# cbg-ethz/LongSom

Measured on AMD Instinct MI355X. Metric: genomic sites/s pileup+call, 10M-read BAM x 5k barcodes, 1/2/4/8 MI355X, higher is better.
Workload: dtype u32

## Files before the change

### longsom_amd/csrc/lsg_api.hip

```cpp
#include "lsg_ctx.h"
#include <cstdarg>
#include <cstring>

namespace lsg {
static thread_local char g_err[512] = "";
void set_error(const char* fmt, ...) {
    va_list ap; va_start(ap, fmt); vsnprintf(g_err, sizeof(g_err), fmt, ap); va_end(ap);
}
const char* get_error() { return g_err; }

int run_count(lsg_ctx* c, const lsg_count_params* p);
int run_fetch_counts(lsg_ctx* c, int ct, int64_t* keys, uint8_t* ref, uint32_t* counts, int64_t capacity);
int run_call(lsg_ctx* c, const lsg_call_params* p);
int run_fetch_calls(lsg_ctx* c, lsg_call* out, int64_t capacity, int candidates_only, int64_t* n_out);
int run_select_calls(lsg_ctx* c, int kind, lsg_call* dst_device, int64_t capacity, int64_t* n_out);
int run_probe(lsg_ctx* c, int kind, const int64_t* keys, int64_t n, uint8_t* hits, int on_device);
int run_set_table_names(lsg_ctx* c, int32_t n_contigs, const char* contig_names, int32_t n_ct, const char* ct_names);
int run_format_table(lsg_ctx* c, int32_t table, int64_t* n_bytes);
int run_copy_table(lsg_ctx* c, int32_t table, char* dst, int64_t capacity);
int run_append_table(lsg_ctx* c, int32_t table, const char* path);
int run_free_table(lsg_ctx* c, int32_t table);
int run_step2_summary(lsg_ctx* c, int32_t n_cols, uint8_t* kinds, int64_t* n_survivor_bytes);
int run_genotype(lsg_ctx* c, const lsg_genotype_params* p, int64_t n_sites, const int64_t* site_keys, const uint8_t* alt_sym,
                 uint32_t* dp, uint32_t* alt, int on_device, int32_t max_depth, int64_t n_groups, const int64_t* group_off);
// ... 35 lines not shown

int lsg_create(int device_id, lsg_ctx** out) {
    if (!out) { set_error("lsg_create: out is NULL"); return -2; }
    *out = nullptr;
    int n = 0;
    if (hipGetDeviceCount(&n) != hipSuccess || n <= 0) {
        set_error("lsg_create: no HIP device visible (this library has no CPU fallback)");
        return -1;
    }
    if (device_id < 0 || device_id >= n) { set_error("lsg_create: device %d out of range [0,%d)", device_id, n); return -2; }
    LSG_HIP(hipSetDevice(device_id));
    lsg_ctx* c = new lsg_ctx();
    c->device = device_id;
    { hipDeviceProp_t prop; if (hipGetDeviceProperties(&prop, device_id) == hipSuccess && prop.multiProcessorCount > 0) c->n_cus = prop.multiProcessorCount; }
    if (hipStreamCreateWithFlags(&c->copy_stream, hipStreamNonBlocking) != hipSuccess || hipEventCreateWithFlags(&c->ev_copy, hipEventDisableTiming) != hipSuccess || hipEventCreateWithFlags(&c->ev_blk, hipEventDisableTiming) != hipSuccess || hipEventCreateWithFlags(&c->ev_lpt, hipEventDisableTiming) != hipSuccess ||
        hipStreamCreateWithFlags(&c->own_stream, hipStreamNonBlocking) != hipSuccess) {
        set_error("lsg_create: hipStreamCreate failed"); delete c; return -1;
    }
    c->stream = c->own_stream;
    if (hipHostMalloc(reinterpret_cast<void**>(&c->h_pin), 4096, hipHostMallocDefault) != hipSuccess) { set_error("lsg_create: hipHostMalloc failed"); delete c; return -1; }
    for (auto& e : c->ev)
        if (hipEventCreate(&e) != hipSuccess) { set_error("lsg_create: hipEventCreate failed"); delete c; return -1; }
    for (auto& e : c->evb)
        if (hipEventCreate(&e) != hipSuccess) { set_error("lsg_create: hipEventCreate failed"); delete c; return -1; }
    *out = c;
    return 0;
}

void lsg_destroy(lsg_ctx* c) {
    if (!c) return;
// ... 11 lines not shown
    for (auto& b : c->syn) b.release();
    for (auto& b : c->gen) b.release();
    (void)run_free_table(c, -1);
    c->cg.release();
    c->tab_names.release();
    for (auto& b : c->ws) b.release();
    for (auto& b : c->tm) b.release();
    for (auto& b : c->bt) b.release();
    for (auto& e : c->ev) if (e) (void)hipEventDestroy(e);
    for (auto& e : c->evb) if (e) (void)hipEventDestroy(e);
    if (c->own_stream) (void)hipStreamDestroy(c->own_stream);
    if (c->copy_stream) (void)hipStreamDestroy(c->copy_stream);
    if (c->ev_copy) (void)hipEventDestroy(c->ev_copy);
    if (c->ev_blk) (void)hipEventDestroy(c->ev_blk);
    if (c->ev_lpt) (void)hipEventDestroy(c->ev_lpt);
    if (c->h_pin) (void)hipHostFree(c->h_pin);
    delete c;
}

int lsg_unload_reads(lsg_ctx* c) {
    if (!c) { set_error("lsg_unload_reads: NULL handle"); return -2; }
    LSG_HIP(hipSetDevice(c->device));
    LSG_HIP(hipStreamSynchronize(c->stream));
    DevBuf* bufs[] = {&c->b_read_tid, &c->b_read_pos, &c->b_read_flag, &c->b_read_mapq, &c->b_read_cb, &c->b_seg_read, &c->b_seg_start, &c->b_seg_len,
                      &c->b_seg_ev_off, &c->b_events, &c->d_read_key, &c->d_read_drop, &c->d_read_adm, &c->d_ne_units, &c->d_ne_mask, &c->d_ne_rowbase, &c->d_ne_rowoff,
                      &c->d_cub_tmp, &c->d_ix_stat, &c->d_tile_cap, &c->d_tile_off, &c->d_calls, &c->d_site_off, &c->d_pass_list, &c->d_defer_list};
    for (auto* b : bufs) b->release();
    for (auto& b : c->d_rows) b.release();
    for (auto& b : c->gen) b.release();
    for (auto& b : c->ws) b.release();
// ... 436 lines not shown
```

### longsom_amd/csrc/lsg_ctx.h

```cpp
#pragma once
#include <hip/hip_runtime.h>
#include <cstdint>
#include <cstdio>
#include <string>
#include <vector>
#include "../../include/longsom_hip.h"
#include "../../include/longsom_synth.h"

namespace lsg {

constexpr int TILE_W = 64;
constexpr int ROW_PLANES = 34;
constexpr int NCTR = 33;

constexpr int ROW_QUADS = (ROW_PLANES + 3) / 4;
constexpr uint64_t ROW_BLOCK_WORDS = (uint64_t)ROW_QUADS * 256;
constexpr uint64_t ROW_STORED_WORDS = (uint64_t)ROW_QUADS * 4;
constexpr uint32_t ROW_NARROW = 1u << 31;
__host__ __device__ inline uint64_t row_word(uint64_t row, int plane) {
    return (row >> 6) * ROW_BLOCK_WORDS + (uint64_t)(plane >> 2) * 256 + (row & 63) * 4 + (uint64_t)(plane & 3);
}

void set_error(const char* fmt, ...);
const char* get_error();
// ... 66 lines not shown
__global__ void k_read_end(const uint32_t* seg_read, const int32_t* seg_start, const int32_t* seg_len, int64_t n_segs, int32_t* read_end);
__global__ void k_read_end_init(const int32_t* read_pos, int64_t n_reads, int32_t* read_end);
int depth_cap_drops(lsg_ctx* c, const lsg_count_params* p);
struct GatherCountSrc { const uint16_t* events; int64_t n_events; const uint64_t* key; const uint32_t* rdv; int32_t cb_bits; int32_t src_shift; int32_t wsh; };
int run_gather_count(lsg_ctx* c, const lsg_count_params* p, const GatherCountSrc& src, bool direct);
}

struct lsg_ctx {
    int device = 0;
    hipStream_t stream = nullptr;
    hipStream_t own_stream = nullptr;
    hipStream_t copy_stream = nullptr;
    hipEvent_t ev_copy = nullptr;
    hipEvent_t ev_blk = nullptr;
    hipEvent_t ev_lpt = nullptr;
    hipEvent_t ev[6] = {nullptr, nullptr, nullptr, nullptr, nullptr, nullptr};
    hipEvent_t evb[5] = {nullptr, nullptr, nullptr, nullptr, nullptr};

    int32_t n_contigs = 0;
    std::vector<int64_t> contig_len;
    std::vector<uint32_t> tile_base;
    uint32_t n_tiles = 0;
    uint32_t tile_lo = 0, tile_hi = 0;
    lsg::DevBuf d_tile_base, d_contig_len, d_ref_ptrs;
    std::vector<lsg::DevBuf> ref;
    std::vector<const uint8_t*> ref_ptr;

    int32_t n_cb = 0, n_ct = 0;
    lsg::DevBuf d_celltype_of, d_ct_rank;
    std::vector<uint8_t> h_celltype_of;
// ... 85 lines not shown
```

### longsom_amd/csrc/pileup.hip

```cpp
#include "lsg_ctx.h"
#include <hipcub/hipcub.hpp>
#include <cstdio>
#include <cstdlib>
#include <cstring>

namespace lsg {

#define LSG_AS3 __attribute__((address_space(3)))
__device__ __forceinline__ uint32_t lds_addr(const void* p) { return (uint32_t)(uintptr_t)(LSG_AS3 const void*)p; }
constexpr int ARENA = 256;

enum { SC_COLS = 8, SC_OVERFLOW = 9, SC_READS = 10, SC_SEGS = 11, SC_EVENTS = 12, SC_ROWS_DEEP = 15,
       SC_ROWS = 16, SC_ROWS_SRC = 28, SC_NENT = 38, SC_QWALK = 48,
       SC_ROWALLOC = 160, SC_ROWALLOC_STRIDE = 16, SC_COUNT = SC_ROWALLOC + SC_ROWALLOC_STRIDE * LSG_MAX_CELLTYPES };

struct CountArgs {
    int64_t n_reads;
    const int32_t* read_tid; const uint16_t* read_flag; const uint8_t* read_mapq; const int32_t* read_cb;
    const int64_t* contig_len; const uint8_t* const* ref_ptr;
    const uint8_t* celltype_of;
    int32_t n_contigs, n_cb, n_ct;
    uint32_t tile_lo, tile_hi;
    int32_t min_bq, min_mq, min_dp, min_cc, ignore_orphans;
    uint32_t flag_exclude;
// ... 1139 lines not shown
            __syncthreads();
            const uint32_t nn = rl(s_q[2], 0);
            const int ct = tm.ct_base + wv;
            if (counting && ct < a.n_ct)
                tm_finish<TmCounters>(a, pl + wv * 1024, nc_sh[wv][lane], cj.w0 + ct, cj.slab + (uint32_t)ct * cj.nj, cj.nj, cj.tcnt, ct, cj.tid, cj.tstart, lane, &book, refb, 0);
            if (nxt == XcdQueue::NO_JOB) break;
            cur = nxt; nxt = nn;
        }
    }
    lds_fence();
    __syncthreads();
    stat_flush(tg.stat_slots, stat, lane, wv);
    books_flush(a, books, lane);
}

__device__ __forceinline__ void tw_add(TmState& s0, TmState& s1, uint32_t m, uint32_t ev, uint32_t thr, uint32_t pk0, uint32_t pk1, uint32_t one) {
    const uint32_t r = m;
    if (!TM_ASM) {
        const uint32_t ln = threadIdx.x & 63u;
        auto half = [&](TmState& s, uint32_t e, uint32_t f, uint32_t inv, uint32_t pk) {
            if (m & TMM_CLOSE) { s.nc += s.mask & 0x10001u; s.mask = 0; }
            if (m & TMM_SKIP) return;
            const bool counted = (e & 0xffu) >= thr && ln >= f && ln < 64u - inv;
            if (!counted) return;
            const uint32_t addr = (pk | (e & 0x700u)) + (m & TMM_CT12);
            const uint32_t sym8 = (e >> 8) & 15u, ctone = 1u << ((m >> 8) & 16u);
            uint32_t hi = 1u;
            if (m & TMM_SINGLE) s.nc += ctone;
            else if (m & TMM_FIRST) s.mask = (1u << sym8) | ctone;
            else { hi |= (s.mask & (1u << sym8)) << 5; s.mask |= (1u << sym8) | ctone; }
            __hip_atomic_fetch_add((LSG_AS3 unsigned long long*)(uintptr_t)addr, ((unsigned long long)hi << 32) | ((e & 0xffu) | (m & TMM_FWD)), __ATOMIC_RELAXED, __HIP_MEMORY_SCOPE_WORKGROUP);
        };
        half(s0, ev & 0xffffu, r & 63u, (r >> 6) & 63u, pk0);
        half(s1, ev >> 16, (r >> 13) & 63u, (r >> 21) & 63u, pk1);
        return;
    }
    uint32_t t0, t1, addr, dlo, elo, ehi, sa, sb, sc, st; unsigned long long xm;
#define TW_RANGE0 "s_lshr_b32 %[st], %[r], 6\n\ts_lshl_b64 %[xm], -1, %[r]\n\ts_lshr_b64 exec, -1, %[st]\n\ts_and_b64 exec, exec, %[xm]\n\t"
#define TW_RANGE1 "s_lshr_b32 %[st], %[r], 13\n\ts_lshl_b64 %[xm], -1, %[st]\n\ts_lshr_b32 %[st], %[r], 21\n\ts_lshr_b64 exec, -1, %[st]\n\ts_and_b64 exec, exec, %[xm]\n\t"
#define TW_HEAD(WSEL, BSEL, PK, DLO)                                                                                                 \
        "v_and_b32_sdwa %[addr], %[c700], %[ev] dst_sel:DWORD dst_unused:UNUSED_PAD src0_sel:DWORD src1_sel:" WSEL "\n\t"           \
        "v_or3_b32 %[addr], %[addr], " PK ", %[sa]\n\t"                                                                             \
        "v_or_b32_sdwa " DLO ", %[sb], %[ev] dst_sel:DWORD dst_unused:UNUSED_PAD src0_sel:DWORD src1_sel:" BSEL "\n\t"              \
        "v_cmpx_le_u32_sdwa vcc, %[thr], %[ev] src0_sel:DWORD src1_sel:" BSEL "\n\t"
    asm volatile(
        "s_bitcmp1_b32 %[m], 27\n\t"
        "s_cbranch_scc0 1f\n\t"
        "v_and_b32 %[t0], 0x10001, %[mask0]\n\t"
        "v_and_b32 %[t1], 0x10001, %[mask1]\n\t"
        "v_add_u32 %[nc0], %[nc0], %[t0]\n\t"
        "v_add_u32 %[nc1], %[nc1], %[t1]\n\t"
        "v_mov_b32 %[mask0], 0\n\t"
        "v_mov_b32 %[mask1], 0\n"
        "1:\n\t"
        "s_bitcmp1_b32 %[m], 29\n\t"
        "s_cbranch_scc1 9f\n\t"
        "s_and_b32 %[sa], %[m], 0x1000\n\t"
        "s_and_b32 %[sb], %[m], 0x100000\n\t"
        "s_lshr_b32 %[sc], %[sa], 8\n\t"
        "s_lshl_b32 %[sc], 1, %[sc]\n\t"
        "s_bitcmp1_b32 %[m], 30\n\t"
        "s_cbranch_scc0 2f\n\t"
        TW_RANGE0
        TW_HEAD("WORD_0", "BYTE_0", "%[pk0]", "v92")
        "ds_add_u64 %[addr], v[92:93]\n\t"
        "v_add_u32 %[nc0], %[sc], %[nc0]\n\t"
        TW_RANGE1
        TW_HEAD("WORD_1", "BYTE_2", "%[pk1]", "v92")
        "ds_add_u64 %[addr], v[92:93]\n\t"
        "v_add_u32 %[nc1], %[sc], %[nc1]\n\t"
        "s_branch 8f\n"
        "2:\n\t"
        "s_bitcmp1_b32 %[m], 28\n\t"
        "s_cbranch_scc0 3f\n\t"
        TW_RANGE0
        TW_HEAD("WORD_0", "BYTE_0", "%[pk0]", "v92")
        "v_bfe_u32 %[t1], %[ev], 8, 4\n\t"
        "ds_add_u64 %[addr], v[92:93]\n\t"
        "v_lshl_or_b32 %[mask0], %[one], %[t1], %[sc]\n\t"
        TW_RANGE1
        TW_HEAD("WORD_1", "BYTE_2", "%[pk1]", "v92")
        "v_bfe_u32 %[t1], %[ev], 24, 4\n\t"
        "ds_add_u64 %[addr], v[92:93]\n\t"
        "v_lshl_or_b32 %[mask1], %[one], %[t1], %[sc]\n\t"
        "s_branch 8f\n"
        "3:\n\t"
        TW_RANGE0
        TW_HEAD("WORD_0", "BYTE_0", "%[pk0]", "v94")
        "v_lshlrev_b32_sdwa %[t1], %[ev], %[one] dst_sel:DWORD dst_unused:UNUSED_PAD src0_sel:BYTE_1 src1_sel:DWORD\n\t"
        "v_and_b32 %[t0], %[mask0], %[t1]\n\t"
        "v_lshl_or_b32 v95, %[t0], 5, %[one]\n\t"
        "ds_add_u64 %[addr], v[94:95]\n\t"
        "v_or3_b32 %[mask0], %[mask0], %[t1], %[sc]\n\t"
        TW_RANGE1
        TW_HEAD("WORD_1", "BYTE_2", "%[pk1]", "v94")
        "v_lshlrev_b32_sdwa %[t1], %[ev], %[one] dst_sel:DWORD dst_unused:UNUSED_PAD src0_sel:BYTE_3 src1_sel:DWORD\n\t"
        "v_and_b32 %[t0], %[mask1], %[t1]\n\t"
        "v_lshl_or_b32 v95, %[t0], 5, %[one]\n\t"
        "ds_add_u64 %[addr], v[94:95]\n\t"
        "v_or3_b32 %[mask1], %[mask1], %[t1], %[sc]\n"
        "8:\n\t"
        "s_mov_b64 exec, -1\n"
        "9:"
        : [t0] "=&v"(t0), [t1] "=&v"(t1), [addr] "=&v"(addr), [dlo] "=&{v92}"(dlo), [elo] "=&{v94}"(elo), [ehi] "=&{v95}"(ehi),
          [sa] "=&s"(sa), [sb] "=&s"(sb), [sc] "=&s"(sc), [st] "=&s"(st), [xm] "=&s"(xm),
          [mask0] "+v"(s0.mask), [nc0] "+v"(s0.nc), [mask1] "+v"(s1.mask), [nc1] "+v"(s1.nc)
        : [ev] "v"(ev), [m] "s"(m), [r] "s"(m), [thr] "s"(thr), [c700] "s"(0x700u), [one] "{v93}"(one), [pk0] "v"(pk0), [pk1] "v"(pk1)
        : "scc", "vcc", "memory");
#undef TW_RANGE0
#undef TW_RANGE1
#undef TW_HEAD
}

struct TwCounters {
    const uint32_t* pl; int lane; uint32_t ncdup;
    __device__ __forceinline__ uint32_t lo(int k) const { return pl[(lane & 1) * 2048 + k * 64 + (lane >> 1) * 2]; }
    __device__ __forceinline__ uint32_t hi(int k) const { return pl[(lane & 1) * 2048 + k * 64 + (lane >> 1) * 2 + 1]; }
    __device__ __forceinline__ uint32_t BC(int k) const { return hi(k) & 0x1fffu; }
    __device__ __forceinline__ uint32_t DUP(int k) const { return hi(k) >> (13 + k); }
    __device__ __forceinline__ uint32_t BQ(int k) const { return lo(k) & 0xfffffu; }
    __device__ __forceinline__ uint32_t BCF(int k) const { return lo(k) >> 20; }
    __device__ __forceinline__ uint32_t NCDUP() const { return ncdup; }
};
struct TwPre { uint32_t bits, ctv, rng; };
#ifndef LSG_TW_GROUP
#define LSG_TW_GROUP 64
// ... 11 lines not shown
    auto load_keys = [&](uint32_t i_first) -> uint64_t {
        const uint32_t i = i_first + (uint32_t)e, ic = i < n ? i : n - 1u;
        return __builtin_nontemporal_load(tg.key + off + ic);
    };
    uint32_t cb_carry = rl((uint32_t)key_before & cbm, 0);
    uint32_t cb_last = 0;
    auto words = [&](int g, uint64_t Kk, TdW& w, TwPre& pre) {
        const uint32_t i = i0 + (uint32_t)TW_G * (uint32_t)g + (uint32_t)e;
        const bool valid = i < i1;
        const uint32_t cb = (uint32_t)Kk & cbm;
        const uint32_t up = (uint32_t)__shfl((int)cb, e ? lane - 1 : lane), dn = (uint32_t)__shfl((int)cb, e < TW_G - 1 ? lane + 1 : lane);
        const uint32_t cb_prev = e == 0 ? cb_carry : up;
        const uint32_t geom = (uint32_t)(Kk >> tg.cb_bits), first = geom & 127u, nev = valid ? ((geom >> 7) & 127u) + 1u : 0u, end = first + nev;
        const uint64_t fld = (Kk >> (tg.cb_bits + 14)) & tg.src_mask;
        const uint64_t addr = evb + (fld << 8);
        const bool rs = i == 0 || cb_prev != cb;
        const bool nd = i + 1 == n || (e < TW_G - 1 && dn != cb);
        w.lo = (uint32_t)addr; w.hi = (uint32_t)(addr >> 32);
        const uint32_t kv = (uint32_t)(Kk >> 32) & (TG_RV_FWD | TG_RV_SEGFIRST);
        pre.ctv = reinterpret_cast<const uint32_t*>(a.celltype_of)[(cb < (uint32_t)a.n_cb ? cb : 0u) >> 2];
        pre.bits = (valid ? 1u : 0u) | (cb < (uint32_t)a.n_cb ? 2u : 0u) | ((kv & TG_RV_FWD) ? 4u : 0u) | (nd ? 8u : 0u) | (rs ? 16u : 0u) |
                   (nev << 16) | ((kv & TG_RV_SEGFIRST) ? (1u << 24) : 0u) | ((cb & 3u) << 26);
        uint32_t f0 = (first + 1u) >> 1, e0 = (end + 1u) >> 1, f1 = first >> 1, e1 = end >> 1;
        if (f0 >= e0) { f0 = 63u; e0 = 1u; }
        if (f1 >= e1) { f1 = 63u; e1 = 1u; }
        pre.rng = f0 | (((64u - e0) & 63u) << 6) | (f1 << 13) | (((64u - e1) & 63u) << 21);
        cb_last = cb_carry = rl(cb, TW_G - 1);
    };
    auto finish_meta = [&](const TwPre& pre, uint32_t cb_of_last, uint32_t cb_after) -> uint32_t {
        if (!(pre.bits & 1u)) return TMM_SKIP;
        uint32_t cls = 2;
        if (pre.bits & 2u) { const uint32_t ct = (pre.ctv >> (((pre.bits >> 26) & 3u) * 8u)) & 0xffu; if (ct < (uint32_t)a.n_ct && (ct >> 1) == (uint32_t)(tm.ct_base >> 1)) cls = ct & 1u; }
        if (cls < 2 && lane < TW_G) { stat.ev += (pre.bits >> 16) & 0xffu; stat.sg += (pre.bits >> 24) & 1u; ++stat.ne; }
        const bool nd = (pre.bits & 8u) != 0 || (e == TW_G - 1 && cb_after != cb_of_last);
        const bool single = (pre.bits & 16u) != 0 && nd;
        uint32_t M = cls < 2 ? (cls ? TMM_CT12 : 0u) | ((pre.bits & 4u) ? TMM_FWD : 0u) | (single ? TMM_SINGLE : 0u) | pre.rng : TMM_SKIP;
        if (pre.bits & 16u) M |= TMM_RS;
        return M;
    };
    uint32_t open_in = 0;
    auto verdicts = [&](uint32_t M) -> uint32_t {
        const bool there = !(M & TMM_SKIP), multi = there && !(M & TMM_SINGLE), rs = (M & TMM_RS) != 0;
        const unsigned long long gm = TW_G == 64 ? ~0ull : 0xffffffffull;
        const unsigned long long A = __ballot(multi) & gm, R = __ballot(rs) & gm;
        const unsigned long long below = (1ull << e) - 1ull;
        const unsigned long long rb = R & below;
        const unsigned long long seg = rb ? below & ~((1ull << (63 - __clzll((long long)rb))) - 1ull) : below;
        const bool ob = (A & seg) != 0ull || (!rb && open_in);
        if (rs && ob) M |= TMM_CLOSE;
        if (multi && (rs || !ob)) M |= TMM_FIRST;
        const unsigned long long segl = R ? ~((1ull << (63 - __clzll((long long)R))) - 1ull) : ~0ull;
        open_in = ((A & segl & gm) != 0ull || (!R && open_in)) ? 1u : 0u;
        return M;
    };
    auto issue_block = [&](const TdW& w, int q, uint32_t (&E)[TD_Q]) {
        uint32_t o = lane4;
        asm volatile("" : "+v"(o));
#pragma unroll
        for (int u0 = 0; u0 < TD_Q; u0 += 8) {
            uint64_t base[8];
#pragma unroll
            for (int u = 0; u < 8; ++u) base[u] = ((uint64_t)rl(w.hi, q * TD_Q + u0 + u) << 32) | rl(w.lo, q * TD_Q + u0 + u);
            asm volatile("" : "+s"(base[0]), "+s"(base[1]), "+s"(base[2]), "+s"(base[3]), "+s"(base[4]), "+s"(base[5]), "+s"(base[6]), "+s"(base[7]));
#pragma unroll
            for (int u = 0; u < 8; ++u)
                E[u0 + u] = *(const __attribute__((address_space(1))) uint32_t*)((const __attribute__((address_space(1))) char*)(uintptr_t)base[u] + (uint64_t)o);
        }
    };
    auto consume = [&](const uint32_t (&E)[TD_Q], int q, uint32_t M) {
#pragma unroll
        for (int u = 0; u < TD_Q; ++u) tw_add(st0, st1, rl(M, q * TD_Q + u), E[u], thr, pkl0, pkl1, one);
    };
    auto fence = []() { asm volatile("" ::: "memory"); };
    uint32_t EA[TD_Q], EB[TD_Q];
    TdW wc, wn; TwPre pre;
    words(0, K, wc, pre);
    fence();
    K = load_keys(i0 + (uint32_t)TW_G);
    fence();
    issue_block(wc, 0, EA);
    fence();
    issue_block(wc, 1, EB);
    fence();
    for (int g = 0; g < ng; ++g) {
        const uint32_t cb_after = rl((uint32_t)K & cbm, 0);
        const uint32_t Mc = verdicts(finish_meta(pre, cb_last, cb_after));
        words(g + 1, K, wn, pre);
        fence();
        K = load_keys(i0 + (uint32_t)TW_G * (uint32_t)(g + 2));
        fence();
#pragma unroll
        for (int sb = 0; sb < TW_NQ; sb += 2) {
            consume(EA, sb, Mc); issue_block(sb + 2 < TW_NQ ? wc : wn, (sb + 2) % TW_NQ, EA);
            consume(EB, sb + 1, Mc); issue_block(sb + 3 < TW_NQ ? wc : wn, (sb + 3) % TW_NQ, EB);
        }
        wc = wn;
    }
    st0.nc += st0.mask & 0x10001u; st0.mask = 0;
    st1.nc += st1.mask & 0x10001u; st1.mask = 0;
}

__global__ __launch_bounds__(TMW_WAVES * 64) __attribute__((amdgpu_waves_per_eu(LSG_TW_WAVES))) void k_tm_count_win(CountArgs a, TmArgs tm, TgArgs tg) {
    __shared__ __attribute__((aligned(16384))) uint32_t planes[2][2][2][8][32][2];
    __shared__ uint32_t nc_sh[2][2][64];
    __shared__ WaveBook books[TMW_WAVES];
    __shared__ uint32_t s_q[4];
    const int lane = threadIdx.x & 63, wv = __builtin_amdgcn_readfirstlane((int)(threadIdx.x >> 6));
    uint32_t* pl = &planes[0][0][0][0][0][0];
    WaveBook& book = books[wv];
// ... 37 lines not shown
                TmState st0, st1; st0.nc = 0; st0.mask = 0; st1.nc = 0; st1.mask = 0;
                tw_range(a, tm, tg, st0, st1, stat, i0, i1, jb.off, jb.tcnt, thr, pkl0, one, lane, K64, kb);
                uint32_t* nq = &nc_sh[0][lane >> 5][2 * (lane & 31)];
                if (st0.nc & 0xffffu) atomicAdd(nq, st0.nc & 0xffffu);
                if (st0.nc >> 16) atomicAdd(nq + 128, st0.nc >> 16);
                if (st1.nc & 0xffffu) atomicAdd(nq + 1, st1.nc & 0xffffu);
                if (st1.nc >> 16) atomicAdd(nq + 129, st1.nc >> 16);
            }
            if (threadIdx.x == 0) s_q[2] = q.answer();
            const JobRec cj = jb;
            jb.load(jw);
            prefetch();
            __syncthreads();
            const uint32_t nn = rl(s_q[2], 0);
            if (mine) {
                for (int v = 0; v < 2; ++v) {
                    const int ct = tm.ct_base + v;
                    if (ct >= a.n_ct) break;
                    const uint32_t uw = (uint32_t)wv * (uint32_t)a.n_ct + (uint32_t)ct;
                    tm_finish<TwCounters>(a, pl + v * 1024 + wv * 512, nc_sh[v][wv][lane], cj.w0 + uw, cj.slab + uw * cj.nj, cj.nj, cj.tcnt, ct, cj.tid, cj.tstart + 64 * wv,
                                          lane, &book, refb, 2 * v);
                }
            }
            if (nxt == XcdQueue::NO_JOB) break;
            cur = nxt; nxt = nn;
        }
    }
    lds_fence();
    __syncthreads();
    stat_flush(tg.stat_slots, stat, lane, wv);
    books_flush(a, books, lane);
}

struct WideEntry {
    bool rs; uint32_t cls; bool fwd;
    uint32_t nev; bool segfirst;
// ... 142 lines not shown
        c->arena = (uint32_t)(arena < (uint64_t)ARENA ? (uint64_t)ARENA : (arena > 8ull * ARENA ? 8ull * ARENA : arena));
        want_rows += emitters * c->arena + 64;
        want_rows = (want_rows + 63) / 64 * 64 + 64;
        if (want_rows > c->row_cap) c->row_cap = want_rows;
        for (int i = 0; i < c->n_ct; ++i)
            if (c->d_rows[i].reserve((size_t)c->row_cap * ROW_STORED_WORDS * 4)) return -1;
    }
    c->n_ne = n_ne; c->n_multi = c->tm_n_multi;
    L.a = CountArgs{};
    fill_args(c, p, L.a);
    TmArgs& tm = L.tm;
    tm = TmArgs{};
    tm.store = c->tm[TM_STORE].as<uint4>(); tm.s0 = c->tm[TM_S0].as<uint32_t>(); tm.b = c->tm[TM_B].as<uint8_t>(); tm.rd = c->tm[TM_RD].as<uint32_t>();
    tm.meta = c->tm[TM_META].as<uint32_t>(); tm.blk_tile = c->tm[TM_BLK_TILE].as<uint32_t>(); tm.jobs = c->tm[TM_JOBS].as<TmJob>(); tm.np = c->tm_np; tm.nblk = c->tm_nblk;
    tm.njobs = c->tm_njobs; tm.nchunks = c->tm_nchunks; tm.chunk_start = c->tm[TM_CHUNKS].as<uint32_t>(); tm.ext = c->tm[TM_EXT].as<uint16_t>();
    LSG_HIP(hipEventRecord(c->ev[0], st));
    {
        PrepArgs pa{}; int k = 0;
        auto op = [&](void* dst, const void* src, size_t bytes) { if (bytes) { pa.op[k].dst = dst; pa.op[k].src = src; pa.op[k].words = (bytes + 3) / 4; ++k; } };
        op(c->d_scalars.p, nullptr, SC_COUNT * 8);
        op(c->d_ix_stat.p, nullptr, IX_STAT_SLOTS * 64);
        if (n_ne) {
            op(c->d_ne_units.p, c->tm[TM_NE_UNITS].p, (size_t)n_ne * 4);
            op(c->ws[WS_NE_GEOM].p, c->tm[TM_NE_GEOM].p, (size_t)n_ne * 8);
            op(c->ws[WS_NE_NSLOT].p, c->tm[TM_NE_NSLOT].p, ((size_t)n_ne + 1) * 4);
            op(c->ws[WS_NE_ACC].p, c->tm[TM_NE_ACC].p, ((size_t)n_ne + 1) * 4);
            if (c->tm_n_multi) op(c->ws[WS_MULTI_LIST].p, c->tm[TM_MULTI].p, (size_t)c->tm_n_multi * 4);
            op(c->d_ne_mask.p, nullptr, ((size_t)n_ne + 1) * 8);
            op(c->d_ne_rowbase.p, nullptr, ((size_t)n_ne + 1) * 4);
        }
        pa.n = k;
        hipLaunchKernelGGL(k_prep_ops, dim3((unsigned)(c->n_cus * 4)), dim3(256), 0, st, pa);
    }
    const int64_t R = c->rd.n_reads;
    if (R > 0) { unsigned g = (unsigned)((R + 255) / 256); if (g > (unsigned)(c->n_cus * 8)) g = (unsigned)(c->n_cus * 8); hipLaunchKernelGGL(k_read_stats, dim3(g), dim3(256), 0, st, L.a); }
    return 0;
}
static int count_passes(lsg_ctx* c, CountLaunch& L, int first_pass, bool wide_of_pass0) {
    hipStream_t st = c->stream;
    const unsigned grid_wide = c->tm_n_wide ? (c->tm_n_wide < (unsigned)(c->n_cus * 4) ? c->tm_n_wide : (unsigned)(c->n_cus * 4)) : 0u;
    for (int pass = wide_of_pass0 ? 0 : first_pass; pass < L.n_pass && c->tm_nblk; ++pass) {
        const bool wide_only = pass < first_pass;
        if (wide_only && !grid_wide) continue;
        L.tm.ct_base = 2 * pass;
        if (pass) LSG_HIP(hipMemsetAsync(L.a.scalars + SC_QWALK, 0, 8, st));
        if (L.a.drop_pairs) hipLaunchKernelGGL(k_tm_resolve<true>, dim3((c->tm_nblk + 255) / 256), dim3(256), 0, st, L.a, L.tm, wide_only ? (unsigned long long*)nullptr : c->d_ix_stat.as<unsigned long long>());
        else hipLaunchKernelGGL(k_tm_resolve<false>, dim3((c->tm_nblk + 255) / 256), dim3(256), 0, st, L.a, L.tm, wide_only ? (unsigned long long*)nullptr : c->d_ix_stat.as<unsigned long long>());
        if (pass == 0) { LSG_HIP(hipEventRecord(c->ev[1], st)); LSG_HIP(hipEventRecord(c->ev[3], st)); }
        if (c->tm_njobs && !wide_only) hipLaunchKernelGGL(k_tm_walk, dim3(L.grid_walk), dim3(TMW_WAVES * 64), 0, st, L.a, L.tm);
        if (pass == 0) LSG_HIP(hipEventRecord(c->ev[4], st));
        if (grid_wide) hipLaunchKernelGGL(k_tm_walk_wide<WideFromStore>, dim3(grid_wide), dim3(64), 0, st, L.a, L.tm, WideFromStore{0}, (const uint32_t*)nullptr);
    }
    return 0;
}
static int count_finish(lsg_ctx* c, const lsg_count_params* p, CountLaunch& L) {
    hipStream_t st = c->stream;
    if (c->tm_nblk) hipLaunchKernelGGL(k_resolve_stats, dim3(1), dim3(256), 0, st, L.a, c->d_ix_stat.as<unsigned long long>());
    if (c->tm_n_multi) hipLaunchKernelGGL(k_finalize_multi, dim3(c->tm_n_multi < L.grid_fin ? c->tm_n_multi : L.grid_fin), dim3(FIN_THREADS), 0, st, L.a);
    LSG_HIP(hipEventRecord(c->ev[5], st));
    LSG_HIP(hipGetLastError());
    unsigned long long sc[SC_COUNT];
    if (read_scalars(c, sc)) return -1;
    if (sc[SC_OVERFLOW]) { set_error("lsg_pileup_count: row buffer overflow (cap %llu)", (unsigned long long)c->row_cap); return -3; }
    for (int i = 0; i < LSG_MAX_CELLTYPES; ++i) c->n_rows[i] = (int64_t)sc[SC_ROWS + i];
    c->n_columns = (int64_t)sc[SC_COLS];
    c->stats.n_reads_admitted = (int64_t)sc[SC_READS];
    c->stats.n_segs_admitted = (int64_t)sc[SC_SEGS];
    c->stats.n_events_admitted = (int64_t)sc[SC_EVENTS];
    c->stats.n_units = c->n_ne;
    c->stats.n_deep_units = c->tm_n_multi;
    c->stats.n_entries = (int64_t)sc[SC_NENT];
    float ms = 0;
    LSG_HIP(hipEventElapsedTime(&ms, c->ev[0], c->ev[1])); c->stats.ms_bin = ms;
// ... 163 lines not shown
```

Measured before the change: 3.551 billion.

## Batch walk atomics per block, drop ballot verdicts, run read stats on side stream

The per-entry tw_add becomes tw_add_batch, which handles sixteen entries per call in one asm block. A run state (sa, sa1, sc) carried across entries replaces the per-group ballot-based verdicts computation, which removes the wave ballots and close/first flag logic. The walk loop now splits into a fully unrolled path for full groups and a nounroll dynamic tail. Separately, k_read_stats is launched on the copy stream with event dependencies so it can overlap the resolve and walk kernels, with a wait added before finish and before the next prep. These changes risk correctness in the run-state semantics and add register pressure from sixteen entries held in asm operands.

Result: faster. 3.593 billion, median of 6 (+1.2%).

```diff
diff --git a/longsom_amd/csrc/lsg_api.hip b/longsom_amd/csrc/lsg_api.hip
--- a/longsom_amd/csrc/lsg_api.hip
+++ b/longsom_amd/csrc/lsg_api.hip
@@ -73,6 +73,7 @@
     c->device = device_id;
     { hipDeviceProp_t prop; if (hipGetDeviceProperties(&prop, device_id) == hipSuccess && prop.multiProcessorCount > 0) c->n_cus = prop.multiProcessorCount; }
     if (hipStreamCreateWithFlags(&c->copy_stream, hipStreamNonBlocking) != hipSuccess || hipEventCreateWithFlags(&c->ev_copy, hipEventDisableTiming) != hipSuccess || hipEventCreateWithFlags(&c->ev_blk, hipEventDisableTiming) != hipSuccess || hipEventCreateWithFlags(&c->ev_lpt, hipEventDisableTiming) != hipSuccess ||
+        hipEventCreateWithFlags(&c->ev_prep, hipEventDisableTiming) != hipSuccess || hipEventCreateWithFlags(&c->ev_rstat, hipEventDisableTiming) != hipSuccess ||
         hipStreamCreateWithFlags(&c->own_stream, hipStreamNonBlocking) != hipSuccess) {
         set_error("lsg_create: hipStreamCreate failed"); delete c; return -1;
     }
@@ -114,6 +115,8 @@
     if (c->ev_copy) (void)hipEventDestroy(c->ev_copy);
     if (c->ev_blk) (void)hipEventDestroy(c->ev_blk);
     if (c->ev_lpt) (void)hipEventDestroy(c->ev_lpt);
+    if (c->ev_prep) (void)hipEventDestroy(c->ev_prep);
+    if (c->ev_rstat) (void)hipEventDestroy(c->ev_rstat);
     if (c->h_pin) (void)hipHostFree(c->h_pin);
     delete c;
 }
diff --git a/longsom_amd/csrc/lsg_ctx.h b/longsom_amd/csrc/lsg_ctx.h
--- a/longsom_amd/csrc/lsg_ctx.h
+++ b/longsom_amd/csrc/lsg_ctx.h
@@ -104,6 +104,8 @@
     hipEvent_t ev_copy = nullptr;
     hipEvent_t ev_blk = nullptr;
     hipEvent_t ev_lpt = nullptr;
+    hipEvent_t ev_prep = nullptr, ev_rstat = nullptr;
+    bool rstat_aside = false;
     hipEvent_t ev[6] = {nullptr, nullptr, nullptr, nullptr, nullptr, nullptr};
     hipEvent_t evb[5] = {nullptr, nullptr, nullptr, nullptr, nullptr};
 
diff --git a/longsom_amd/csrc/pileup.hip b/longsom_amd/csrc/pileup.hip
--- a/longsom_amd/csrc/pileup.hip
+++ b/longsom_amd/csrc/pileup.hip
@@ -1177,102 +1177,120 @@
     books_flush(a, books, lane);
 }
 
-__device__ __forceinline__ void tw_add(TmState& s0, TmState& s1, uint32_t m, uint32_t ev, uint32_t thr, uint32_t pk0, uint32_t pk1, uint32_t one) {
-    const uint32_t r = m;
+struct TwRun { uint32_t sa, sa1, sc; };
+template <bool DYN>
+__device__ __forceinline__ void tw_add_batch(TmState& s0, TmState& s1, TwRun& run, uint32_t M, int l0, const uint32_t (&E)[TD_Q], uint32_t thr, uint32_t pk0, uint32_t pk1, uint32_t one) {
     if (!TM_ASM) {
         const uint32_t ln = threadIdx.x & 63u;
-        auto half = [&](TmState& s, uint32_t e, uint32_t f, uint32_t inv, uint32_t pk) {
-            if (m & TMM_CLOSE) { s.nc += s.mask & 0x10001u; s.mask = 0; }
-            if (m & TMM_SKIP) return;
-            const bool counted = (e & 0xffu) >= thr && ln >= f && ln < 64u - inv;
-            if (!counted) return;
-            const uint32_t addr = (pk | (e & 0x700u)) + (m & TMM_CT12);
-            const uint32_t sym8 = (e >> 8) & 15u, ctone = 1u << ((m >> 8) & 16u);
-            uint32_t hi = 1u;
-            if (m & TMM_SINGLE) s.nc += ctone;
-            else if (m & TMM_FIRST) s.mask = (1u << sym8) | ctone;
-            else { hi |= (s.mask & (1u << sym8)) << 5; s.mask |= (1u << sym8) | ctone; }
-            __hip_atomic_fetch_add((LSG_AS3 unsigned long long*)(uintptr_t)addr, ((unsigned long long)hi << 32) | ((e & 0xffu) | (m & TMM_FWD)), __ATOMIC_RELAXED, __HIP_MEMORY_SCOPE_WORKGROUP);
-        };
-        half(s0, ev & 0xffffu, r & 63u, (r >> 6) & 63u, pk0);
-        half(s1, ev >> 16, (r >> 13) & 63u, (r >> 21) & 63u, pk1);
+        for (int u = 0; u < TD_Q; ++u) {
+            const uint32_t r = rl(M, l0 + u);
+            if (r & TMM_RS) {
+                s0.nc += s0.mask & 0x10001u; s0.mask = 0; s1.nc += s1.mask & 0x10001u; s1.mask = 0;
+                if (r & TMM_SKIP) continue;
+                run.sa = r & TMM_CT12; run.sc = 1u << (run.sa >> 8);
+            }
+            auto half = [&](TmState& s, uint32_t e, uint32_t f, uint32_t inv, uint32_t pk) {
+                const bool counted = (e & 0xffu) >= thr && ln >= f && ln < 64u - inv;
+                if (!counted) return;
+                const uint32_t addr = (pk | (e & 0x700u)) + run.sa;
+                const uint32_t symbit = 1u << ((e >> 8) & 15u);
+                uint32_t hi = 1u;
+                if ((r & TMM_RS) && (r & TMM_SINGLE)) s.nc += run.sc;
+                else { hi |= (s.mask & symbit) << 5; s.mask |= symbit | run.sc; }
+                __hip_atomic_fetch_add((LSG_AS3 unsigned long long*)(uintptr_t)addr, ((unsigned long long)hi << 32) | ((e & 0xffu) | (r & TMM_FWD)), __ATOMIC_RELAXED, __HIP_MEMORY_SCOPE_WORKGROUP);
+            };
+            half(s0, E[u] & 0xffffu, r & 63u, (r >> 6) & 63u, pk0);
+            half(s1, E[u] >> 16, (r >> 13) & 63u, (r >> 21) & 63u, pk1);
+        }
         return;
     }
-    uint32_t t0, t1, addr, dlo, elo, ehi, sa, sb, sc, st; unsigned long long xm;
-#define TW_RANGE0 "s_lshr_b32 %[st], %[r], 6\n\ts_lshl_b64 %[xm], -1, %[r]\n\ts_lshr_b64 exec, -1, %[st]\n\ts_and_b64 exec, exec, %[xm]\n\t"
-#define TW_RANGE1 "s_lshr_b32 %[st], %[r], 13\n\ts_lshl_b64 %[xm], -1, %[st]\n\ts_lshr_b32 %[st], %[r], 21\n\ts_lshr_b64 exec, -1, %[st]\n\ts_and_b64 exec, exec, %[xm]\n\t"
-#define TW_HEAD(WSEL, BSEL, PK, DLO)                                                                                                 \
-        "v_and_b32_sdwa %[addr], %[c700], %[ev] dst_sel:DWORD dst_unused:UNUSED_PAD src0_sel:DWORD src1_sel:" WSEL "\n\t"           \
-        "v_or3_b32 %[addr], %[addr], " PK ", %[sa]\n\t"                                                                             \
-        "v_or_b32_sdwa " DLO ", %[sb], %[ev] dst_sel:DWORD dst_unused:UNUSED_PAD src0_sel:DWORD src1_sel:" BSEL "\n\t"              \
-        "v_cmpx_le_u32_sdwa vcc, %[thr], %[ev] src0_sel:DWORD src1_sel:" BSEL "\n\t"
-    asm volatile(
-        "s_bitcmp1_b32 %[m], 27\n\t"
-        "s_cbranch_scc0 1f\n\t"
-        "v_and_b32 %[t0], 0x10001, %[mask0]\n\t"
-        "v_and_b32 %[t1], 0x10001, %[mask1]\n\t"
-        "v_add_u32 %[nc0], %[nc0], %[t0]\n\t"
-        "v_add_u32 %[nc1], %[nc1], %[t1]\n\t"
-        "v_mov_b32 %[mask0], 0\n\t"
-        "v_mov_b32 %[mask1], 0\n"
-        "1:\n\t"
-        "s_bitcmp1_b32 %[m], 29\n\t"
-        "s_cbranch_scc1 9f\n\t"
-        "s_and_b32 %[sa], %[m], 0x1000\n\t"
-        "s_and_b32 %[sb], %[m], 0x100000\n\t"
-        "s_lshr_b32 %[sc], %[sa], 8\n\t"
-        "s_lshl_b32 %[sc], 1, %[sc]\n\t"
-        "s_bitcmp1_b32 %[m], 30\n\t"
-        "s_cbranch_scc0 2f\n\t"
-        TW_RANGE0
-        TW_HEAD("WORD_0", "BYTE_0", "%[pk0]", "v92")
-        "ds_add_u64 %[addr], v[92:93]\n\t"
-        "v_add_u32 %[nc0], %[sc], %[nc0]\n\t"
-        TW_RANGE1
-        TW_HEAD("WORD_1", "BYTE_2", "%[pk1]", "v92")
-        "ds_add_u64 %[addr], v[92:93]\n\t"
-        "v_add_u32 %[nc1], %[sc], %[nc1]\n\t"
-        "s_branch 8f\n"
-        "2:\n\t"
-        "s_bitcmp1_b32 %[m], 28\n\t"
-        "s_cbranch_scc0 3f\n\t"
-        TW_RANGE0
-        TW_HEAD("WORD_0", "BYTE_0", "%[pk0]", "v92")
-        "v_bfe_u32 %[t1], %[ev], 8, 4\n\t"
-        "ds_add_u64 %[addr], v[92:93]\n\t"
-        "v_lshl_or_b32 %[mask0], %[one], %[t1], %[sc]\n\t"
-        TW_RANGE1
-        TW_HEAD("WORD_1", "BYTE_2", "%[pk1]", "v92")
-        "v_bfe_u32 %[t1], %[ev], 24, 4\n\t"
-        "ds_add_u64 %[addr], v[92:93]\n\t"
-        "v_lshl_or_b32 %[mask1], %[one], %[t1], %[sc]\n\t"
-        "s_branch 8f\n"
-        "3:\n\t"
-        TW_RANGE0
-        TW_HEAD("WORD_0", "BYTE_0", "%[pk0]", "v94")
-        "v_lshlrev_b32_sdwa %[t1], %[ev], %[one] dst_sel:DWORD dst_unused:UNUSED_PAD src0_sel:BYTE_1 src1_sel:DWORD\n\t"
-        "v_and_b32 %[t0], %[mask0], %[t1]\n\t"
-        "v_lshl_or_b32 v95, %[t0], 5, %[one]\n\t"
-        "ds_add_u64 %[addr], v[94:95]\n\t"
-        "v_or3_b32 %[mask0], %[mask0], %[t1], %[sc]\n\t"
-        TW_RANGE1
-        TW_HEAD("WORD_1", "BYTE_2", "%[pk1]", "v94")
-        "v_lshlrev_b32_sdwa %[t1], %[ev], %[one] dst_sel:DWORD dst_unused:UNUSED_PAD src0_sel:BYTE_3 src1_sel:DWORD\n\t"
-        "v_and_b32 %[t0], %[mask1], %[t1]\n\t"
-        "v_lshl_or_b32 v95, %[t0], 5, %[one]\n\t"
-        "ds_add_u64 %[addr], v[94:95]\n\t"
-        "v_or3_b32 %[mask1], %[mask1], %[t1], %[sc]\n"
-        "8:\n\t"
-        "s_mov_b64 exec, -1\n"
-        "9:"
-        : [t0] "=&v"(t0), [t1] "=&v"(t1), [addr] "=&v"(addr), [dlo] "=&{v92}"(dlo), [elo] "=&{v94}"(elo), [ehi] "=&{v95}"(ehi),
-          [sa] "=&s"(sa), [sb] "=&s"(sb), [sc] "=&s"(sc), [st] "=&s"(st), [xm] "=&s"(xm),
-          [mask0] "+v"(s0.mask), [nc0] "+v"(s0.nc), [mask1] "+v"(s1.mask), [nc1] "+v"(s1.nc)
-        : [ev] "v"(ev), [m] "s"(m), [r] "s"(m), [thr] "s"(thr), [c700] "s"(0x700u), [one] "{v93}"(one), [pk0] "v"(pk0), [pk1] "v"(pk1)
-        : "scc", "vcc", "memory");
+    static_assert(!TM_ASM || TD_Q == 16, "tw_add_batch's asm spells sixteen entries out");
+    uint32_t t0, t1, addr, dlo, elo, ehi, sb, st, m; unsigned long long xm;
+#define TW_M(K) "%[m]"
+#define TW_E(K) "%[e" #K "]"
+#define TW_RANGE0(K) "s_lshr_b32 %[st], " TW_M(K) ", 6\n\ts_lshl_b64 %[xm], -1, " TW_M(K) "\n\ts_lshr_b64 exec, -1, %[st]\n\ts_and_b64 exec, exec, %[xm]\n\t"
+#define TW_RANGE1(K) "s_lshr_b32 %[st], " TW_M(K) ", 13\n\ts_lshl_b64 %[xm], -1, %[st]\n\ts_lshr_b32 %[st], " TW_M(K) ", 21\n\ts_lshr_b64 exec, -1, %[st]\n\ts_and_b64 exec, exec, %[xm]\n\t"
+#define TW_HEAD(K, WSEL, BSEL, SA, DLO)                                                                                              \
+        "v_and_b32_sdwa %[addr], %[c700], " TW_E(K) " dst_sel:DWORD dst_unused:UNUSED_PAD src0_sel:DWORD src1_sel:" WSEL "\n\t"       \
+        "v_or3_b32 %[addr], %[addr], %[pk0], " SA "\n\t"                                                                            \
+        "v_or_b32_sdwa " DLO ", %[sb], " TW_E(K) " dst_sel:DWORD dst_unused:UNUSED_PAD src0_sel:DWORD src1_sel:" BSEL "\n\t"          \
+        "v_cmpx_le_u32_sdwa vcc, %[thr], " TW_E(K) " src0_sel:DWORD src1_sel:" BSEL "\n\t"
+#define TW_BODY(K, N)                                                                                                                \
+        TW_RL(N)                                                                                                                     \
+        "s_bitcmp1_b32 " TW_M(K) ", 31\n\t"                                                                                          \
+        "s_cbranch_scc1 1" #K "f\n"                                                                                                  \
+        "2" #K ":\n\t"                                                                                                               \
+        "s_and_b32 %[sb], " TW_M(K) ", 0x100000\n\t"                                                           \
+        TW_RANGE0(K)                                                                                                                 \
+        TW_HEAD(K, "WORD_0", "BYTE_0", "%[sa]", "v94")                                                                              \
+        "v_lshlrev_b32_sdwa %[t1], " TW_E(K) ", %[one] dst_sel:DWORD dst_unused:UNUSED_PAD src0_sel:BYTE_1 src1_sel:DWORD\n\t"       \
+        "v_and_b32 %[t0], %[mask0], %[t1]\n\t"                                          \
+        "v_lshl_or_b32 v95, %[t0], 5, %[one]\n\t"                                                                                    \
+        "ds_add_u64 %[addr], v[94:95]\n\t"                                                                                           \
+        "v_or3_b32 %[mask0], %[mask0], %[t1], %[sc]\n\t"                                                                             \
+        TW_RANGE1(K)                                                                                                                 \
+        TW_HEAD(K, "WORD_1", "BYTE_2", "%[sa1]", "v94")                                                                              \
+        "v_lshlrev_b32_sdwa %[t1], " TW_E(K) ", %[one] dst_sel:DWORD dst_unused:UNUSED_PAD src0_sel:BYTE_3 src1_sel:DWORD\n\t"      \
+        "v_and_b32 %[t0], %[mask1], %[t1]\n\t"                                                                                       \
+        "v_lshl_or_b32 v95, %[t0], 5, %[one]\n\t"                                                                                    \
+        "ds_add_u64 %[addr], v[94:95]\n\t"                                                                                           \
+        "v_or3_b32 %[mask1], %[mask1], %[t1], %[sc]\n\t"                                                                             \
+        "s_mov_b64 exec, -1\n"                                                                                                       \
+        "3" #K ":\n\t"
+#define TW_START(K, N)                                                                                                               \
+        "1" #K ":\n\t"                                                                                                               \
+        "v_and_b32 %[t0], 0x10001, %[mask0]\n\t"                                \
+        "v_and_b32 %[t1], 0x10001, %[mask1]\n\t"                                                                                     \
+        "v_add_u32 %[nc0], %[nc0], %[t0]\n\t"                                                                                        \
+        "v_add_u32 %[nc1], %[nc1], %[t1]\n\t"                                                                                        \
+        "v_mov_b32 %[mask0], 0\n\t"                                                                                                  \
+        "v_mov_b32 %[mask1], 0\n\t"                                                                                                  \
+        "s_bitcmp1_b32 " TW_M(K) ", 29\n\t"                                                                                          \
+        "s_cbranch_scc1 3" #K "b\n\t"                                                                 \
+        "s_and_b32 %[sa], " TW_M(K) ", 0x1000\n\t"                                                   \
+        "s_or_b32 %[sa1], %[sa], 0x2000\n\t"                                                                                       \
+        "s_lshr_b32 %[sc], %[sa], 8\n\t"                                                                                             \
+        "s_lshl_b32 %[sc], 1, %[sc]\n\t"                                         \
+        "s_bitcmp1_b32 " TW_M(K) ", 30\n\t"                                                                                          \
+        "s_cbranch_scc0 2" #K "b\n\t"                               \
+        "s_and_b32 %[sb], " TW_M(K) ", 0x100000\n\t"                                                  \
+        TW_RANGE0(K)                                                                                                                 \
+        TW_HEAD(K, "WORD_0", "BYTE_0", "%[sa]", "v92")                                                                              \
+        "ds_add_u64 %[addr], v[92:93]\n\t"                                                                                           \
+        "v_add_u32 %[nc0], %[sc], %[nc0]\n\t"                                                                                        \
+        TW_RANGE1(K)                                                                                                                 \
+        TW_HEAD(K, "WORD_1", "BYTE_2", "%[sa1]", "v92")                                                                              \
+        "ds_add_u64 %[addr], v[92:93]\n\t"                                                                                           \
+        "v_add_u32 %[nc1], %[sc], %[nc1]\n\t"                                                                                        \
+        "s_mov_b64 exec, -1\n\t"                                                                                                     \
+        "s_branch 3" #K "b\n"
+#define TW_ALL(F) F(00, 0) F(01, 1) F(02, 2) F(03, 3) F(04, 4) F(05, 5) F(06, 6) F(07, 7) F(08, 8) F(09, 9) F(10, 10) F(11, 11) F(12, 12) F(13, 13) F(14, 14) F(15, 15)
+#define TW_OPERANDS(L0)                                                                                                              \
+        : [t0] "=&v"(t0), [t1] "=&v"(t1), [addr] "=&v"(addr), [dlo] "=&{v92}"(dlo), [elo] "=&{v94}"(elo), [ehi] "=&{v95}"(ehi),        \
+          [sb] "=&s"(sb), [st] "=&s"(st), [xm] "=&s"(xm), [m] "=&s"(m), [sa] "+s"(run.sa), [sa1] "+s"(run.sa1), [sc] "+s"(run.sc),                          \
+          [mask0] "+v"(s0.mask), [nc0] "+v"(s0.nc), [mask1] "+v"(s1.mask), [nc1] "+v"(s1.nc)                                         \
+        : [e00] "v"(E[0]), [e01] "v"(E[1]), [e02] "v"(E[2]), [e03] "v"(E[3]), [e04] "v"(E[4]), [e05] "v"(E[5]), [e06] "v"(E[6]), [e07] "v"(E[7]),            \
+          [e08] "v"(E[8]), [e09] "v"(E[9]), [e10] "v"(E[10]), [e11] "v"(E[11]), [e12] "v"(E[12]), [e13] "v"(E[13]), [e14] "v"(E[14]), [e15] "v"(E[15]),    \
+          [M] "v"(M), L0, [thr] "s"(thr), [c700] "s"(0x700u), [one] "{v93}"(one), [pk0] "v"(pk0)                   \
+        : "scc", "vcc", "memory"
+    if (DYN) {
+#define TW_RL(N) "s_add_u32 %[st], %[l0], " #N "\n\tv_readlane_b32 %[m], %[M], %[st]\n\t"
+        asm volatile(TW_ALL(TW_BODY) "s_branch 9f\n" TW_ALL(TW_START) "9:" TW_OPERANDS([l0] "s"(l0)));
+#undef TW_RL
+    } else {
+#define TW_RL(N) "v_readlane_b32 %[m], %[M], %[l0]+" #N "\n\t"
+        asm volatile(TW_ALL(TW_BODY) "s_branch 9f\n" TW_ALL(TW_START) "9:" TW_OPERANDS([l0] "n"(l0)));
+#undef TW_RL
+    }
+#undef TW_OPERANDS
+#undef TW_ALL
+#undef TW_START
+#undef TW_BODY
+#undef TW_HEAD
+#undef TW_RANGE1
 #undef TW_RANGE0
-#undef TW_RANGE1
-#undef TW_HEAD
+#undef TW_E
+#undef TW_M
 }
 
 struct TwCounters {
@@ -1314,7 +1332,7 @@
         const uint32_t geom = (uint32_t)(Kk >> tg.cb_bits), first = geom & 127u, nev = valid ? ((geom >> 7) & 127u) + 1u : 0u, end = first + nev;
         const uint64_t fld = (Kk >> (tg.cb_bits + 14)) & tg.src_mask;
         const uint64_t addr = evb + (fld << 8);
-        const bool rs = i == 0 || cb_prev != cb;
+        const bool rs = i == i0 || cb_prev != cb;
         const bool nd = i + 1 == n || (e < TW_G - 1 && dn != cb);
         w.lo = (uint32_t)addr; w.hi = (uint32_t)(addr >> 32);
         const uint32_t kv = (uint32_t)(Kk >> 32) & (TG_RV_FWD | TG_RV_SEGFIRST);
@@ -1328,30 +1346,14 @@
         cb_last = cb_carry = rl(cb, TW_G - 1);
     };
     auto finish_meta = [&](const TwPre& pre, uint32_t cb_of_last, uint32_t cb_after) -> uint32_t {
-        if (!(pre.bits & 1u)) return TMM_SKIP;
+        if (!(pre.bits & 1u)) return TMM_SKIP | TMM_RS;
         uint32_t cls = 2;
         if (pre.bits & 2u) { const uint32_t ct = (pre.ctv >> (((pre.bits >> 26) & 3u) * 8u)) & 0xffu; if (ct < (uint32_t)a.n_ct && (ct >> 1) == (uint32_t)(tm.ct_base >> 1)) cls = ct & 1u; }
         if (cls < 2 && lane < TW_G) { stat.ev += (pre.bits >> 16) & 0xffu; stat.sg += (pre.bits >> 24) & 1u; ++stat.ne; }
+        if (cls == 2) return TMM_SKIP | TMM_RS;
         const bool nd = (pre.bits & 8u) != 0 || (e == TW_G - 1 && cb_after != cb_of_last);
         const bool single = (pre.bits & 16u) != 0 && nd;
-        uint32_t M = cls < 2 ? (cls ? TMM_CT12 : 0u) | ((pre.bits & 4u) ? TMM_FWD : 0u) | (single ? TMM_SINGLE : 0u) | pre.rng : TMM_SKIP;
-        if (pre.bits & 16u) M |= TMM_RS;
-        return M;
-    };
-    uint32_t open_in = 0;
-    auto verdicts = [&](uint32_t M) -> uint32_t {
-        const bool there = !(M & TMM_SKIP), multi = there && !(M & TMM_SINGLE), rs = (M & TMM_RS) != 0;
-        const unsigned long long gm = TW_G == 64 ? ~0ull : 0xffffffffull;
-        const unsigned long long A = __ballot(multi) & gm, R = __ballot(rs) & gm;
-        const unsigned long long below = (1ull << e) - 1ull;
-        const unsigned long long rb = R & below;
-        const unsigned long long seg = rb ? below & ~((1ull << (63 - __clzll((long long)rb))) - 1ull) : below;
-        const bool ob = (A & seg) != 0ull || (!rb && open_in);
-        if (rs && ob) M |= TMM_CLOSE;
-        if (multi && (rs || !ob)) M |= TMM_FIRST;
-        const unsigned long long segl = R ? ~((1ull << (63 - __clzll((long long)R))) - 1ull) : ~0ull;
-        open_in = ((A & segl & gm) != 0ull || (!R && open_in)) ? 1u : 0u;
-        return M;
+        return (cls ? TMM_CT12 : 0u) | ((pre.bits & 4u) ? TMM_FWD : 0u) | (single ? TMM_SINGLE : 0u) | ((pre.bits & 16u) ? TMM_RS : 0u) | pre.rng;
     };
     auto issue_block = [&](const TdW& w, int q, uint32_t (&E)[TD_Q]) {
         uint32_t o = lane4;
@@ -1367,32 +1369,62 @@
                 E[u0 + u] = *(const __attribute__((address_space(1))) uint32_t*)((const __attribute__((address_space(1))) char*)(uintptr_t)base[u] + (uint64_t)o);
         }
     };
-    auto consume = [&](const uint32_t (&E)[TD_Q], int q, uint32_t M) {
-#pragma unroll
-        for (int u = 0; u < TD_Q; ++u) tw_add(st0, st1, rl(M, q * TD_Q + u), E[u], thr, pkl0, pkl1, one);
-    };
+    TwRun run; run.sa = 0; run.sa1 = 8192u; run.sc = 1u;
+    auto consume = [&](const uint32_t (&E)[TD_Q], int q, uint32_t M) { tw_add_batch<false>(st0, st1, run, M, q * TD_Q, E, thr, pkl0, pkl1, one); };
+    auto consume_dyn = [&](const uint32_t (&E)[TD_Q], int q, uint32_t M) { tw_add_batch<true>(st0, st1, run, M, q * TD_Q, E, thr, pkl0, pkl1, one); };
     auto fence = []() { asm volatile("" ::: "memory"); };
+    const uint32_t cnt = i1 - i0;
+    const int nfull = (int)(cnt / (uint32_t)TW_G);
     uint32_t EA[TD_Q], EB[TD_Q];
     TdW wc, wn; TwPre pre;
     words(0, K, wc, pre);
+    wn = wc;
     fence();
     K = load_keys(i0 + (uint32_t)TW_G);
     fence();
-    issue_block(wc, 0, EA);
-    fence();
-    issue_block(wc, 1, EB);
-    fence();
-    for (int g = 0; g < ng; ++g) {
+    int g = 0;
+    if (nfull >= 2) {
+        issue_block(wc, 0, EA);
+        fence();
+        issue_block(wc, 1, EB);
+        fence();
+        for (; g + 1 < nfull; ++g) {
+            const uint32_t cb_after = rl((uint32_t)K & cbm, 0);
+            const uint32_t Mc = finish_meta(pre, cb_last, cb_after);
+            words(g + 1, K, wn, pre);
+            fence();
+            K = load_keys(i0 + (uint32_t)TW_G * (uint32_t)(g + 2));
+            fence();
+#pragma unroll
+            for (int sb = 0; sb < TW_NQ; sb += 2) {
+                consume(EA, sb, Mc); issue_block(sb + 2 < TW_NQ ? wc : wn, (sb + 2) % TW_NQ, EA);
+                consume(EB, sb + 1, Mc); issue_block(sb + 3 < TW_NQ ? wc : wn, (sb + 3) % TW_NQ, EB);
+            }
+            wc = wn;
+        }
+    }
+    const int nbt = (int)((cnt - (uint32_t)TW_G * (uint32_t)g + (uint32_t)TD_Q - 1u) / (uint32_t)TD_Q);
+    if (g == 0) {
+        issue_block(wc, 0, EA);
+        if (nbt > 1) issue_block(wc, 1, EB);
+    }
+#pragma nounroll
+    for (int b0 = 0; g < ng; ++g, b0 += TW_NQ) {
         const uint32_t cb_after = rl((uint32_t)K & cbm, 0);
-        const uint32_t Mc = verdicts(finish_meta(pre, cb_last, cb_after));
-        words(g + 1, K, wn, pre);
-        fence();
-        K = load_keys(i0 + (uint32_t)TW_G * (uint32_t)(g + 2));
-        fence();
-#pragma unroll
-        for (int sb = 0; sb < TW_NQ; sb += 2) {
-            consume(EA, sb, Mc); issue_block(sb + 2 < TW_NQ ? wc : wn, (sb + 2) % TW_NQ, EA);
-            consume(EB, sb + 1, Mc); issue_block(sb + 3 < TW_NQ ? wc : wn, (sb + 3) % TW_NQ, EB);
+        const uint32_t Mc = finish_meta(pre, cb_last, cb_after);
+        if (g + 1 < ng) {
+            words(g + 1, K, wn, pre);
+            fence();
+            K = load_keys(i0 + (uint32_t)TW_G * (uint32_t)(g + 2));
+            fence();
+        }
+        const int nbg = nbt - b0 < TW_NQ ? nbt - b0 : TW_NQ;
+#pragma nounroll
+        for (int h = 0; h < nbg; h += 2) {
+            consume_dyn(EA, h, Mc);
+            if (b0 + h + 2 < nbt) issue_block(h + 2 < TW_NQ ? wc : wn, (h + 2) % TW_NQ, EA);
+            if (h + 1 < nbg) consume_dyn(EB, h + 1, Mc);
+            if (b0 + h + 3 < nbt) issue_block(h + 3 < TW_NQ ? wc : wn, (h + 3) % TW_NQ, EB);
         }
         wc = wn;
     }
@@ -1460,12 +1492,14 @@
             __syncthreads();
             const uint32_t nn = rl(s_q[2], 0);
             if (mine) {
+                int lane_f = lane;
+                asm volatile("" : "+v"(lane_f));
                 for (int v = 0; v < 2; ++v) {
                     const int ct = tm.ct_base + v;
                     if (ct >= a.n_ct) break;
                     const uint32_t uw = (uint32_t)wv * (uint32_t)a.n_ct + (uint32_t)ct;
                     tm_finish<TwCounters>(a, pl + v * 1024 + wv * 512, nc_sh[v][wv][lane], cj.w0 + uw, cj.slab + uw * cj.nj, cj.nj, cj.tcnt, ct, cj.tid, cj.tstart + 64 * wv,
-                                          lane, &book, refb, 2 * v);
+                                          lane_f, &book, refb, 2 * v);
                 }
             }
             if (nxt == XcdQueue::NO_JOB) break;
@@ -1638,6 +1672,7 @@
     tm.store = c->tm[TM_STORE].as<uint4>(); tm.s0 = c->tm[TM_S0].as<uint32_t>(); tm.b = c->tm[TM_B].as<uint8_t>(); tm.rd = c->tm[TM_RD].as<uint32_t>();
     tm.meta = c->tm[TM_META].as<uint32_t>(); tm.blk_tile = c->tm[TM_BLK_TILE].as<uint32_t>(); tm.jobs = c->tm[TM_JOBS].as<TmJob>(); tm.np = c->tm_np; tm.nblk = c->tm_nblk;
     tm.njobs = c->tm_njobs; tm.nchunks = c->tm_nchunks; tm.chunk_start = c->tm[TM_CHUNKS].as<uint32_t>(); tm.ext = c->tm[TM_EXT].as<uint16_t>();
+    if (c->rstat_aside) { LSG_HIP(hipStreamWaitEvent(st, c->ev_rstat, 0)); c->rstat_aside = false; }
     LSG_HIP(hipEventRecord(c->ev[0], st));
     {
         PrepArgs pa{}; int k = 0;
@@ -1657,7 +1692,17 @@
         hipLaunchKernelGGL(k_prep_ops, dim3((unsigned)(c->n_cus * 4)), dim3(256), 0, st, pa);
     }
     const int64_t R = c->rd.n_reads;
-    if (R > 0) { unsigned g = (unsigned)((R + 255) / 256); if (g > (unsigned)(c->n_cus * 8)) g = (unsigned)(c->n_cus * 8); hipLaunchKernelGGL(k_read_stats, dim3(g), dim3(256), 0, st, L.a); }
+    if (R > 0) {
+        unsigned g = (unsigned)((R + 255) / 256); if (g > (unsigned)(c->n_cus * 8)) g = (unsigned)(c->n_cus * 8);
+        hipStream_t rs = st;
+        if (!L.a.adm && c->copy_stream && c->ev_prep && c->ev_rstat) {
+            rs = c->copy_stream;
+            LSG_HIP(hipEventRecord(c->ev_prep, st));
+            LSG_HIP(hipStreamWaitEvent(rs, c->ev_prep, 0));
+        }
+        hipLaunchKernelGGL(k_read_stats, dim3(g), dim3(256), 0, rs, L.a);
+        if (rs != st) { LSG_HIP(hipEventRecord(c->ev_rstat, rs)); c->rstat_aside = true; }
+    }
     return 0;
 }
 static int count_passes(lsg_ctx* c, CountLaunch& L, int first_pass, bool wide_of_pass0) {
@@ -1681,6 +1726,7 @@
     hipStream_t st = c->stream;
     if (c->tm_nblk) hipLaunchKernelGGL(k_resolve_stats, dim3(1), dim3(256), 0, st, L.a, c->d_ix_stat.as<unsigned long long>());
     if (c->tm_n_multi) hipLaunchKernelGGL(k_finalize_multi, dim3(c->tm_n_multi < L.grid_fin ? c->tm_n_multi : L.grid_fin), dim3(FIN_THREADS), 0, st, L.a);
+    if (c->rstat_aside) { LSG_HIP(hipStreamWaitEvent(st, c->ev_rstat, 0)); c->rstat_aside = false; }
     LSG_HIP(hipEventRecord(c->ev[5], st));
     LSG_HIP(hipGetLastError());
     unsigned long long sc[SC_COUNT];
```
